# MAC-VO/MAC-VO

Measured on NVIDIA H100. Metric: stereo frames/sec @640x480, higher is better.
Workload: dtype f32

## Files before the change

### include/macvo_b200.h

```cpp
#ifndef MACVO_B200_H
#define MACVO_B200_H

#include <stddef.h>
#include <stdint.h>

#ifdef __cplusplus
extern "C" {
#endif

#define MACVO_OK 0
#define MACVO_E_ARG (-1)
#define MACVO_E_WORKSPACE (-2)
#define MACVO_E_UNSUPPORTED (-3)
#define MACVO_E_DRIVER (-4)

const char* macvo_b200_version(void);

#define MACVO_CORR_SIMT 0
#define MACVO_CORR_TC_3XF16 1
#define MACVO_CORR_TC_1XF16 2
#define MACVO_CORR_TC_TF32 3
#define MACVO_CORR_KMAJOR_INPUT 16
size_t macvo_corr_workspace_bytes(int batch, int dim, int n, int mode);
int macvo_corr_build(const float* fmap1, const float* fmap2, float* corr, int batch, int dim, int n, int mode,
// ... 87 lines not shown
int macvo_p2p_alloc(size_t bytes, void** dev_ptr, unsigned char* ipc_handle64);
int macvo_p2p_open(const unsigned char* ipc_handle64, void** peer_ptr);
int macvo_p2p_close(void* peer_ptr);
int macvo_p2p_free(void* dev_ptr);
int macvo_pgo_solve_sharded(const double* pos_Tw, const double* kp2_uv, const double* kp2_disp, const double* uv_cov,
                            const double* disp_cov, int k_shard, const int* k_total_dev, int k_offset, int min_k,
                            const double* intr, double* pose_io, const macvo_pgo_params_t* params, double* stats,
                            void* const* exchange_bufs, int world, int rank, void* stream);

#define MACVO_PGO_ACC 55
#define MACVO_PGO_MAX_RANKS 8
int macvo_pgo_accumulate(const double* pos_Tw, const double* kp2_uv, const double* kp2_disp, const double* uv_cov,
                         const double* disp_cov, int k, const double* intr, const double* pose, double huber_delta,
                         double* acc, void* stream);

int macvo_layer_norm(const float* x, const float* weight, const float* bias, float* y, long long rows,
                     int channels, float eps, void* stream);
int macvo_add_layer_norm(const float* x, const float* resid, const float* weight, const float* bias, float* sum_out,
                         float* y, long long rows, int channels, float eps, void* stream);
int macvo_mlp_tc(const float* xn, const float* resid, const float* w1, const float* b1, const float* w2, const float* b2,
                 float* out, int rows, int channels, int hidden, void* stream);
int macvo_patch_tokens_tc(const float* x, const float* w0, const float* term, const float* w2, const float* b2,
                          const float* ln_w, const float* ln_b, float* out, long long rows, int in_channels, int channels,
                          int period, float eps, void* stream);
int macvo_patch_embed_conv1(const float* maps, const float* weight, const float* bias, float* out,
                            long long n_maps, int h, int w, int allow_tf32, void* stream);
int macvo_add_rows_relu(float* x, const float* term, long long rows, int period, int channels, void* stream);
int macvo_small_attention(const float* q, const float* k, const float* v, float* out, int batch, int nq, int nk,
                          int heads, int head_dim, int q_broadcast, int allow_tf32, void* stream);

int macvo_small_attention_ex(const float* q, const float* k, const float* v, float* out, int batch, int nq, int nk,
                             int heads, int head_dim, int q_broadcast, int allow_tf32, int ldq, int ldk, int ldv,
                             const float* q_add, const float* k_add, int add_period, void* stream);

int macvo_latent_pool(const float* tokens, const float* ut, const float* wv, const float* bv, float* out,
                      long long n_maps, int nk, void* stream);

int macvo_gru_input(const float* mf, const float* agg, const float* gamma, float* buf0, float* buf1, float* buf2,
                    float* buf3, long long pixels, void* stream);
int macvo_gru_gates(const float* zr, const float* bias, const float* hx, float* z_out, float* rhx, long long pixels,
                    void* stream);
int macvo_gru_blend(const float* q, const float* bias, const float* z, float* hx, float* h_dense, long long pixels,
                    void* stream);
size_t macvo_rows_count(int batch, int height, int width, int vertical);
int macvo_conv_tc(const void* in_rows, int in_channels, int in_dense, const void* weights, const float* bias, int n_pad,
                  int n_valid, int ksize, int relu, int batch, int height, int width, void* out16, int out16_pitch,
                  int out16_offset, int out16_dense, float* out32, int out32_pitch, int out32_offset, int out32_planes,
                  void* stream);
int macvo_flow_im2col(const float* coords1, const float* coords0, void* rows, float* mf32, void* mf16_rows, int batch,
                      int height, int width, void* stream);

size_t macvo_gru_tc_operand_rows(int batch, int height, int width, int vertical);
int macvo_gru_tc_stage(int stage, int vertical, int batch, int height, int width, const void* h_rows, const void* x_rows,
                       const void* weights, const float* bias, float* h_master, float* z, void* out_rows, void* stream);
int macvo_gru_tc_pack(const float* src, int src_pitch, int channels, void* dst, int dst_channels, int dst_offset, int batch,
                      int height, int width, int vertical, void* stream);
int macvo_gru_tc_pack_motion(const float* mf, const float* agg, const float* gamma, void* x_rows_h, void* x_rows_v, int batch,
                             int height, int width, void* stream);
int macvo_softmax_rows_f16(const float* scores, void* out, long long rows, int cols, void* stream);
int macvo_convex_upsample(const float* flow, const float* mask_nhwc, float* out, float scale, int batch, int height, int width,
                          void* stream);

int macvo_cov_sanity_filter(const double* obs1_cov, const double* obs2_cov, int k, uint8_t* good, void* stream);
#define MACVO_COV_MATCH 0
#define MACVO_COV_IDENTITY 1
#define MACVO_COV_GAUSSIAN_MIXTURE 2
// ... 55 lines not shown
```

### mac-vo_b200/csrc/nn_kernels.cu

```cuda
#include "common.cuh"
#include "layer_norm_row.cuh"
#include <math_constants.h>

namespace {

__device__ __forceinline__ float2 ffma2_rn(float2 a, float2 b, float2 c) { return make_float2(fmaf(a.x, b.x, c.x), fmaf(a.y, b.y, c.y)); }
__device__ __forceinline__ float2 fmul2_rn(float2 a, float2 b) { return make_float2(__fmul_rn(a.x, b.x), __fmul_rn(a.y, b.y)); }

template <int VPL>
__global__ void __launch_bounds__(256)
layer_norm_kernel(const float* __restrict__ x, const float* __restrict__ w, const float* __restrict__ b,
                  float* __restrict__ y, long long rows, float eps, const float* __restrict__ resid = nullptr,
                  float* __restrict__ sum_out = nullptr) {
    constexpr int C = 32 * VPL;
    const long long row = (long long)blockIdx.x * 8 + (threadIdx.x >> 5);
    const int lane = threadIdx.x & 31;
    if (row >= rows) return;
    const float* xr = x + row * C;
    float v[VPL];
#pragma unroll
    for (int i = 0; i < VPL / 4; ++i) {
        float4 t = *reinterpret_cast<const float4*>(xr + (lane + 32 * i) * 4);
        if (resid) {
            const float4 r = *reinterpret_cast<const float4*>(resid + row * C + (lane + 32 * i) * 4);
// ... 472 lines not shown
        }
    }
    l0 += __shfl_xor_sync(0xffffffffu, l0, 1); l0 += __shfl_xor_sync(0xffffffffu, l0, 2);
    l1 += __shfl_xor_sync(0xffffffffu, l1, 1); l1 += __shfl_xor_sync(0xffffffffu, l1, 2);
    const float i0 = 1.f / l0, i1 = 1.f / l1;
    const int h0 = 2 * warp, h1 = h0 + 1;
    float o0[2][4], o1[2][4];
#pragma unroll
    for (int nt = 0; nt < 2; ++nt) { o0[nt][0] = o0[nt][1] = o0[nt][2] = o0[nt][3] = 0.f; o1[nt][0] = o1[nt][1] = o1[nt][2] = o1[nt][3] = 0.f; }
#pragma unroll
    for (int nd = 0; nd < KS; ++nd) {
        const uint32_t za[4] = {to_tf32(acc[nd][0] * i0), to_tf32(acc[nd][2] * i1), to_tf32(acc[nd][1] * i0), to_tf32(acc[nd][3] * i1)};
#pragma unroll
        for (int nt = 0; nt < 2; ++nt) {
            const float* w0 = wv + (long long)(h0 * LP_HD + nt * 8 + g) * LP_D + nd * 8 + 2 * t;
            const float* w1 = wv + (long long)(h1 * LP_HD + nt * 8 + g) * LP_D + nd * 8 + 2 * t;
            mma_tf32(o0[nt], za, to_tf32(__ldg(w0)), to_tf32(__ldg(w0 + 1)));
            mma_tf32(o1[nt], za, to_tf32(__ldg(w1)), to_tf32(__ldg(w1 + 1)));
        }
    }
    float* ob = out + (b * 8 + g) * (LP_HEADS * LP_HD);
#pragma unroll
    for (int nt = 0; nt < 2; ++nt) {
        const int d = nt * 8 + 2 * t;
        *reinterpret_cast<float2*>(ob + h0 * LP_HD + d) = make_float2(o0[nt][0] + __ldg(bv + h0 * LP_HD + d), o0[nt][1] + __ldg(bv + h0 * LP_HD + d + 1));
        *reinterpret_cast<float2*>(ob + h1 * LP_HD + d) = make_float2(o1[nt][2] + __ldg(bv + h1 * LP_HD + d), o1[nt][3] + __ldg(bv + h1 * LP_HD + d + 1));
    }
}

constexpr int FQ_HEADS = 8, FQ_SLOTS = 4, FQ_QPT = 2;
template <int FQ_D>
__global__ void __launch_bounds__(128)
attn_few_queries_kernel(const float* __restrict__ q, const float* __restrict__ k, const float* __restrict__ v,
                        float* __restrict__ out, long long batch, int nq, int nk, long long q_bstride, float scale) {
    const long long b = (long long)blockIdx.x * 4 + (threadIdx.x >> 5);
    if (b >= batch) return;
    const int lane = threadIdx.x & 31, hd = lane & 7, slot = lane >> 3;
    constexpr int C = FQ_HEADS * FQ_D;
    float2 qr[FQ_QPT][FQ_D / 2], acc[FQ_QPT][FQ_D / 2];
    float m[FQ_QPT], l[FQ_QPT];
#pragma unroll
    for (int t = 0; t < FQ_QPT; ++t) {
        const int i = min(slot + FQ_SLOTS * t, nq - 1);
        const float* qp = q + b * q_bstride + ((long long)i * FQ_HEADS + hd) * FQ_D;
#pragma unroll
        for (int c = 0; c < FQ_D / 4; ++c) {
            const float4 x = *reinterpret_cast<const float4*>(qp + 4 * c);
            qr[t][2 * c] = make_float2(x.x * scale, x.y * scale);
            qr[t][2 * c + 1] = make_float2(x.z * scale, x.w * scale);
        }
#pragma unroll
        for (int c = 0; c < FQ_D / 2; ++c) acc[t][c] = make_float2(0.f, 0.f);
        m[t] = -CUDART_INF_F; l[t] = 0.f;
    }
    const float4* kp = reinterpret_cast<const float4*>(k + b * nk * C + hd * FQ_D);
    const float4* vp = reinterpret_cast<const float4*>(v + b * nk * C + hd * FQ_D);
#pragma unroll 2
    for (int j = 0; j < nk; ++j) {
        float4 kk[FQ_D / 4], vv[FQ_D / 4];
#pragma unroll
        for (int c = 0; c < FQ_D / 4; ++c) { kk[c] = __ldg(kp + j * (C / 4) + c); vv[c] = __ldg(vp + j * (C / 4) + c); }
#pragma unroll
        for (int t = 0; t < FQ_QPT; ++t) {
            float2 sx = make_float2(0.f, 0.f);
#pragma unroll
            for (int c = 0; c < FQ_D / 4; ++c) {
                sx = ffma2_rn(qr[t][2 * c], make_float2(kk[c].x, kk[c].y), sx);
                sx = ffma2_rn(qr[t][2 * c + 1], make_float2(kk[c].z, kk[c].w), sx);
            }
            const float s = sx.x + sx.y;
            const float mn = fmaxf(m[t], s);
            const float corr = __expf(m[t] - mn), p = __expf(s - mn);
            m[t] = mn;
            l[t] = l[t] * corr + p;
            const float2 c2 = make_float2(corr, corr), p2 = make_float2(p, p);
#pragma unroll
            for (int c = 0; c < FQ_D / 4; ++c) {
                acc[t][2 * c] = ffma2_rn(p2, make_float2(vv[c].x, vv[c].y), fmul2_rn(acc[t][2 * c], c2));
                acc[t][2 * c + 1] = ffma2_rn(p2, make_float2(vv[c].z, vv[c].w), fmul2_rn(acc[t][2 * c + 1], c2));
            }
        }
    }
#pragma unroll
    for (int t = 0; t < FQ_QPT; ++t) {
        const int i = slot + FQ_SLOTS * t;
        if (i >= nq) continue;
        const float inv = 1.f / l[t];
        float* op = out + ((b * nq + i) * FQ_HEADS + hd) * FQ_D;
#pragma unroll
        for (int c = 0; c < FQ_D / 4; ++c)
            *reinterpret_cast<float4*>(op + 4 * c) = make_float4(acc[t][2 * c].x * inv, acc[t][2 * c].y * inv,
                                                                 acc[t][2 * c + 1].x * inv, acc[t][2 * c + 1].y * inv);
    }
}

template <int D>
__global__ void __launch_bounds__(256)
attn_single_query_kernel(const float* __restrict__ q, const float* __restrict__ k, const float* __restrict__ v,
                         float* __restrict__ out, long long batch, int nk, int heads, float scale) {
    const long long e = (long long)blockIdx.x * blockDim.x + threadIdx.x;
    if (e >= batch * heads) return;
    const long long b = e / heads;
    const int hd = (int)(e % heads), C = heads * D;
    float qr[D], acc[D];
#pragma unroll
    for (int c = 0; c < D; c += 4) {
        const float4 t = *reinterpret_cast<const float4*>(q + b * C + hd * D + c);
        qr[c] = t.x * scale; qr[c + 1] = t.y * scale; qr[c + 2] = t.z * scale; qr[c + 3] = t.w * scale;
        acc[c] = acc[c + 1] = acc[c + 2] = acc[c + 3] = 0.f;
    }
    float m = -CUDART_INF_F, l = 0.f;
    const float* kp = k + b * nk * C + hd * D;
    const float* vp = v + b * nk * C + hd * D;
#pragma unroll 4
    for (int j = 0; j < nk; ++j) {
        float kk[D], vv[D];
#pragma unroll
        for (int c = 0; c < D; c += 4) {
            const float4 t = __ldg(reinterpret_cast<const float4*>(kp + (long long)j * C + c));
            const float4 u = __ldg(reinterpret_cast<const float4*>(vp + (long long)j * C + c));
            kk[c] = t.x; kk[c + 1] = t.y; kk[c + 2] = t.z; kk[c + 3] = t.w;
// ... 67 lines not shown
        return MACVO_OK;
    }
    float* packed = nullptr;
    MACVO_CUDA_TRY(cudaGetSymbolAddress(reinterpret_cast<void**>(&packed), g_pe_pack));
    pe_pack_weights_kernel<<<3, 256, 0, st>>>(weight, bias, packed);
    MACVO_LAUNCH_CHECK();
    MACVO_CUDA_TRY(cudaMemcpyToSymbolAsync(c_pe_w, packed, sizeof(float) * (PE_K * PE_K * PE_C + PE_C), 0,
                                           cudaMemcpyDeviceToDevice, st));
    MACVO_CUDA_TRY(cudaFuncSetAttribute(patch_conv1_kernel, cudaFuncAttributeMaxDynamicSharedMemorySize, (int)smem));
    const int items = ho * (wo / 2);
    patch_conv1_kernel<<<(unsigned)n_maps, items % 320 == 0 ? 320 : 256, smem, st>>>(maps, out, h, w, ho, wo);
    MACVO_LAUNCH_CHECK();
    return MACVO_OK;
}

extern "C" int macvo_small_attention_ex(const float* q, const float* k, const float* v, float* out, int batch, int nq,
                                        int nk, int heads, int head_dim, int q_broadcast, int allow_tf32, int ldq, int ldk,
                                        int ldv, const float* q_add, const float* k_add, int add_period, void* stream) {
    if (!q || !k || !v || !out || batch <= 0 || nq <= 0 || nk <= 0 || heads <= 0) return MACVO_E_ARG;
    if (head_dim != 8 && head_dim != 16 && head_dim != 32) return MACVO_E_UNSUPPORTED;
    const int c = heads * head_dim;
    AttnExtra ex{ldq > 0 ? ldq : c, ldk > 0 ? ldk : c, ldv > 0 ? ldv : c, add_period > 0 ? add_period : 1, q_add, k_add};
    const bool plain = ex.ldq == c && ex.ldk == c && ex.ldv == c && !q_add && !k_add;
    if ((ex.ldq | ex.ldk | ex.ldv) & 3) return MACVO_E_ARG;
    cudaStream_t st = as_stream(stream);
    const float scale = 1.f / sqrtf((float)head_dim);
    const long long qbs = q_broadcast ? 0 : (long long)nq * ex.ldq;
    if (plain && nq == 1 && !q_broadcast && head_dim <= 16) {
        const unsigned grid = (unsigned)(((long long)batch * heads + 255) / 256);
        if (head_dim == 16) attn_single_query_kernel<16><<<grid, 256, 0, st>>>(q, k, v, out, batch, nk, heads, scale);
        else attn_single_query_kernel<8><<<grid, 256, 0, st>>>(q, k, v, out, batch, nk, heads, scale);
    } else if (plain && nq <= FQ_SLOTS * FQ_QPT && heads == FQ_HEADS && head_dim <= 16) {
        const unsigned grid = (unsigned)((batch + 3) / 4);
        if (head_dim == 16) attn_few_queries_kernel<16><<<grid, 128, 0, st>>>(q, k, v, out, batch, nq, nk, qbs, scale);
        else attn_few_queries_kernel<8><<<grid, 128, 0, st>>>(q, k, v, out, batch, nq, nk, qbs, scale);
    } else if (head_dim == 8) {
        return MACVO_E_UNSUPPORTED;
    } else if (allow_tf32 && nq >= 16) {
        const size_t smem = (size_t)((nk + 31) / 32 * 32) * ((head_dim / 32) * 32 + 16 + head_dim) * sizeof(float);
        if (smem > 200 * 1024) return MACVO_E_UNSUPPORTED;
        const int warps = nq > 64 ? 8 : 4;
        dim3 grid(ceil_div(nq, 16 * warps), heads, batch);
        if (head_dim == 16) {
            MACVO_CUDA_TRY(cudaFuncSetAttribute(attn_tc_kernel<16>, cudaFuncAttributeMaxDynamicSharedMemorySize, (int)smem));
            attn_tc_kernel<16><<<grid, 32 * warps, smem, st>>>(q, k, v, out, nq, nk, heads, qbs, scale, ex);
        } else {
            MACVO_CUDA_TRY(cudaFuncSetAttribute(attn_tc_kernel<32>, cudaFuncAttributeMaxDynamicSharedMemorySize, (int)smem));
            attn_tc_kernel<32><<<grid, 32 * warps, smem, st>>>(q, k, v, out, nq, nk, heads, qbs, scale, ex);
        }
    } else {
        const size_t smem = (size_t)2 * ((nk + ATT_CHUNK - 1) / ATT_CHUNK * ATT_CHUNK) * head_dim * sizeof(float);
        if (smem > 200 * 1024) return MACVO_E_UNSUPPORTED;
        dim3 grid(ceil_div(nq, 128), heads, batch);
        if (head_dim == 16) {
            MACVO_CUDA_TRY(cudaFuncSetAttribute(attn_shared_kv_kernel<16>, cudaFuncAttributeMaxDynamicSharedMemorySize, (int)smem));
            attn_shared_kv_kernel<16><<<grid, 128, smem, st>>>(q, k, v, out, nq, nk, heads, qbs, scale, ex);
        } else {
            MACVO_CUDA_TRY(cudaFuncSetAttribute(attn_shared_kv_kernel<32>, cudaFuncAttributeMaxDynamicSharedMemorySize, (int)smem));
            attn_shared_kv_kernel<32><<<grid, 128, smem, st>>>(q, k, v, out, nq, nk, heads, qbs, scale, ex);
        }
    }
    MACVO_LAUNCH_CHECK();
    return MACVO_OK;
}

extern "C" int macvo_small_attention(const float* q, const float* k, const float* v, float* out, int batch, int nq,
                                     int nk, int heads, int head_dim, int q_broadcast, int allow_tf32, void* stream) {
    return macvo_small_attention_ex(q, k, v, out, batch, nq, nk, heads, head_dim, q_broadcast, allow_tf32, 0, 0, 0, nullptr,
                                    nullptr, 0, stream);
}

extern "C" int macvo_add_rows_relu(float* x, const float* term, long long rows, int period, int channels, void* stream) {
    if (!x || !term || rows < 0 || period <= 0 || channels <= 0 || (channels & 3)) return MACVO_E_ARG;
    if (rows == 0) return MACVO_OK;
    const long long n = rows * (channels / 4);
    add_rows_relu_kernel<<<(unsigned)((n + 255) / 256), 256, 0, as_stream(stream)>>>(x, term, rows, period, channels / 4);
    MACVO_LAUNCH_CHECK();
    return MACVO_OK;
}

extern "C" int macvo_latent_pool(const float* tokens, const float* ut, const float* wv, const float* bv, float* out,
                                 long long n_maps, int nk, void* stream) {
    if (!tokens || !ut || !wv || !bv || !out || n_maps < 0 || nk <= 0) return MACVO_E_ARG;
    if (n_maps == 0) return MACVO_OK;
    const size_t smem = (size_t)((nk + 31) / 32 * 32) * (LP_D + 4) * sizeof(float);
    if (smem > 200 * 1024) return MACVO_E_UNSUPPORTED;
    MACVO_CUDA_TRY(cudaFuncSetAttribute(latent_pool_kernel, cudaFuncAttributeMaxDynamicSharedMemorySize, (int)smem));
    latent_pool_kernel<<<(unsigned)n_maps, 128, smem, as_stream(stream)>>>(tokens, ut, wv, bv, out, nk);
    MACVO_LAUNCH_CHECK();
    return MACVO_OK;
}
```

### mac-vo_b200/flowformer_cov.py

```python
from __future__ import annotations

import math
import os
import zlib
from typing import Callable

import torch
import torch.nn.functional as F

Tensor = torch.Tensor

LATENT_TOKENS = 8
LATENT_DIM = 128
QUERY_DIM = 64
COST_INPUT_DIM = 64
VERT_C_DIM = 64
ENCODER_DEPTH = 3


def _svt_spec(prefix: str) -> list[tuple[str, tuple[int, ...], str]]:
    out: list[tuple[str, tuple[int, ...], str]] = []
    dims, heads, srs, patch, cin = (128, 256), (4, 8), (8, 4), (4, 2), (3, 128)
    for s, (C, sr, ps, ci) in enumerate(zip(dims, srs, patch, cin)):
        p = f"{prefix}.svt."
# ... 348 lines not shown
                x = self._ops.patch_embed_conv1(cost_maps, self.W[p + "proj.0.weight"], self.W[p + "proj.0.bias"])
                x = self._conv_relu(x, p + "proj.2", stride=2, padding=2)
        else:
            x = F.pad(cost_maps, (0, (8 - W2 % 8) % 8, 0, (8 - H2 % 8) % 8))
            x = self._conv_relu(x, p + "proj.0", stride=2, padding=2)
            x = self._conv_relu(x, p + "proj.2", stride=2, padding=2)
        native = self._native(x)
        x = F.conv2d(x if x.is_contiguous(memory_format=torch.channels_last) else x.contiguous(memory_format=torch.channels_last),
                     self.W[p + "proj.4.weight"], None if native else self.W[p + "proj.4.bias"], stride=2, padding=2)
        h, w = x.shape[2:]

        w0, b0 = self.W[p + "ffn_with_coord.0.weight"], self.W[p + "ffn_with_coord.0.bias"]

        def coord_term():
            xy = coords_grid(1, h, w, x.device, x.dtype) * 8 + 4
            enc = sine_embed(xy.view(1, 2, -1).permute(0, 2, 1), COST_INPUT_DIM)
            term = F.linear(enc, w0[:, COST_INPUT_DIM:, 0, 0], b0)
            if native:
                term = term + F.linear(self.W[p + "proj.4.bias"], w0[:, :COST_INPUT_DIM, 0, 0])
            return term.contiguous()
        term = self._memo(("pe", h, w, x.dtype, x.device, native), coord_term)
        t = x.permute(0, 2, 3, 1).reshape(M, h * w, COST_INPUT_DIM)
        w2 = self.W[p + "ffn_with_coord.2.weight"][:, :, 0, 0]
        if native and torch.backends.cuda.matmul.allow_tf32:
            w0t, w2t = self._memo(("pe_tc", x.device), lambda: (self._ops.round_tf32(w0[:, :COST_INPUT_DIM, 0, 0]),
                                                                self._ops.round_tf32(w2)))
            return self._ops.patch_tokens_tc(t, w0t, term[0], w2t, self.W[p + "ffn_with_coord.2.bias"],
                                             self.W[p + "norm.weight"], self.W[p + "norm.bias"])
        t = F.linear(t, w0[:, :COST_INPUT_DIM, 0, 0])
        t = self._ops.add_rows_relu_(t, term[0]) if native else F.relu(t + term)
        t = F.linear(t, w2, self.W[p + "ffn_with_coord.2.bias"])
        return self._ln(t, p + "norm")

    def _latent_layer(self, x: Tensor, p: str) -> Tensor:
        y = self._ln(x, p + "norm1")
        a = self._attn(self._lin(y, p + "q"), self._lin(y, p + "k"), self._lin(y, p + "v"), 8)
        x, xn = self._add_ln(x, self._lin(a, p + "proj"), p + "norm2")
        return self._mlp_residual(x, xn, p, "ffn.0", "ffn.3")

    def _context_tokens(self, context: Tensor, p: str, reps: int) -> Tensor:
        b, _, H, W = context.shape
        c = self._lin(context.flatten(2).permute(0, 2, 1), p + "context_proj").view(b, H, W, -1)
        return c.repeat(reps, 1, 1, 1)

    def _vert_local_attn_native(self, x: Tensor, size, context: Tensor, p: str, ws: int, heads: int) -> Tensor:
        Bt, N, C = x.shape
        H, W = size
        b = context.shape[0]
        wq, wk = self.W[p + "q.weight"], self.W[p + "k.weight"]
        enc = self._memo(("win", ws, C + VERT_C_DIM, x.dtype, x.device), lambda: sine_embed(
            coords_grid(1, ws, ws, x.device, x.dtype).view(1, 2, -1).permute(0, 2, 1), C + VERT_C_DIM))
        cproj = self._lin(context.flatten(2).permute(0, 2, 1), p + "context_proj").view(b, H, W, -1)
        cw, meta = self._to_windows(cproj, ws)
        w_qk_c = torch.cat([wq[:, C:], wk[:, C:]], 0)
        w_qk = torch.cat([wq, wk], 0)
        b_qk = torch.cat([self.W[p + "q.bias"], self.W[p + "k.bias"]], 0)
        terms = F.linear(cw, w_qk_c) + F.linear(enc, w_qk, b_qk)
        q_add, k_add = terms[..., :C].contiguous(), terms[..., C:].contiguous()
        w_x = self._memo(("vloc_w", p), lambda: torch.cat([wq[:, :C], wk[:, :C], self.W[p + "v.weight"]], 0).contiguous())
        b_x = self._memo(("vloc_b", p), lambda: torch.cat([torch.zeros(2 * C, device=x.device, dtype=x.dtype), self.W[p + "v.bias"]], 0))
        xw, meta = self._to_windows(x.view(Bt, H, W, C), ws)
        qkv = F.linear(xw, w_x, b_x)
        o = self._ops.fused_qkv_attention(qkv, heads, q_add, k_add)
        return self._lin(self._from_windows(o, meta, ws, H, W), p + "proj")

    def _vert_local_attn(self, x: Tensor, size, context: Tensor, p: str, ws: int = 7, heads: int = 8) -> Tensor:
        if self._native(x) and (x.shape[-1] // heads) in (16, 32):
            return self._vert_local_attn_native(x, size, context, p, ws, heads)
        Bt, N, C = x.shape
        H, W = size
        ctx = self._context_tokens(context, p, Bt // context.shape[0])
# ... 51 lines not shown
        k_in = self._conv(qk.permute(0, 3, 1, 2), p + "sr_key", stride=sr).reshape(Bt, C, -1).permute(0, 2, 1)
        v_in, k_in = self._ln(v_in, p + "norm"), self._ln(k_in, p + "norm")
        enc_sub = self._memo(("sub", Hp // sr, Wp // sr, sr, C, x.dtype, x.device), lambda: sine_embed(
            coords_grid(1, Hp // sr, Wp // sr, x.device, x.dtype).view(1, 2, -1).permute(0, 2, 1) * sr, C))
        o = self._attn(q, self._lin(k_in + enc_sub, p + "k"), self._lin(v_in, p + "v"), heads)
        o = o.view(Bt, Hp, Wp, C)[:, :H, :W, :].reshape(Bt, N, C)
        return self._lin(o, p + "proj")

    def _vert_block(self, x: Tensor, size, context: Tensor, p: str, local: bool) -> Tensor:
        attn = self._vert_local_attn if local else self._vert_global_attn
        x, xn = self._add_ln(x, attn(self._ln(x, p + "norm1"), size, context, p + "attn."), p + "norm2")
        return self._mlp_residual(x, xn, p + "mlp.", "fc1", "fc2")

    def cost_perceiver(self, cost_volume: Tensor, context: Tensor) -> tuple[Tensor, Tensor]:
        c = "memory_encoder.cost_perceiver_encoder."
        B, heads, H1, W1, H2, W2 = cost_volume.shape
        assert heads == 1
        cost_maps = cost_volume.view(B * H1 * W1, 1, H2, W2)
        tokens = self.patch_embed(cost_maps)
        p = c + "input_layer."
        lat = self.W[c + "latent_tokens"]
        M = tokens.shape[0]
        q = self._lin(self._ln(lat, p + "norm1"), p + "q")
        if self._native(tokens) and torch.backends.cuda.matmul.allow_tf32 and LATENT_DIM == 128 and LATENT_TOKENS == 8:
            a = self._ops.latent_pool(tokens, q[0], self.W[p + "k.weight"], self.W[p + "v.weight"], self.W[p + "v.bias"])
        else:
            a = self._attn(q, self._lin(tokens, p + "k"), self._lin(tokens, p + "v"), 8)
        x = lat + self._lin(a, p + "proj")
        x = self._mlp_residual(x, self._ln(x, p + "norm2"), p, "ffn.0", "ffn.3")
        short_cut = x
        N = H1 * W1
        self._join_context()
        for i in range(ENCODER_DEPTH):
            x = self._latent_layer(x, c + f"encoder_layers.{i}.")
            x = x.view(B, N, LATENT_TOKENS, -1).permute(0, 2, 1, 3).reshape(B * LATENT_TOKENS, N, -1)
            v_ = c + f"vertical_encoder_layers.{i}."
            x = self._vert_block(x, (H1, W1), context, v_ + "local_block.", True)
            x = self._vert_block(x, (H1, W1), context, v_ + "global_block.", False)
            x = x.view(B, LATENT_TOKENS, N, -1).permute(0, 2, 1, 3).reshape(B * N, LATENT_TOKENS, -1)
        return x + short_cut, cost_maps

    def memory_encoder(self, img1: Tensor, img2: Tensor, context: Tensor, shared: tuple[int, int] | None = None) -> tuple[Tensor, Tensor]:
        B = img1.shape[0]
        if shared is None:
            feats = self.svt(torch.cat([img1, img2], dim=0), "memory_encoder.feat_encoder")
            feats = self._conv(feats, "memory_encoder.channel_convertor")
            f1, f2 = feats[:B], feats[B:]
        else:
            i, j = shared
            if not (0 <= i < B and 0 <= j < B):
                raise ValueError(f"shared={shared}: image indices must lie in [0, {B})")
            keep = [k for k in range(B) if k != j]
            feats = self.svt(torch.cat([img1] + [img2[k:k + 1] for k in keep], dim=0), "memory_encoder.feat_encoder")
            feats = self._conv(feats, "memory_encoder.channel_convertor")
            f1 = feats[:B]
            f2 = torch.empty_like(f1)
            for pos, k in enumerate(keep):
                f2[k:k + 1].copy_(feats[B + pos:B + pos + 1])
            f2[j:j + 1].copy_(feats[i:i + 1])
            if self.taps is not None:
                feats = torch.cat([f1, f2], dim=0)
        self._tap("feats", feats)
        cost_volume = self.corr_fn(f1, f2).to(feats.dtype)
        self._tap("corr_rows", cost_volume.reshape(B, -1, cost_volume.shape[-2] * cost_volume.shape[-1])[:, ::97])
        out = self.cost_perceiver(cost_volume, context)
        self._tap("cost_memory", out[0])
        return out

    def _gru(self, h: Tensor, x: Tensor, p: str) -> Tensor:
        for o, pad in (("1", (0, 2)), ("2", (2, 0))):
            hx = torch.cat([h, x], dim=1)
            zr = torch.sigmoid(self._conv(hx, p + f"convzr{o}", padding=pad))
# ... 316 lines not shown
```

### mac-vo_b200/ops.py

```python
from __future__ import annotations

import ctypes as C
import os
import threading

import torch

from .build import LIB_PATH

Tensor = torch.Tensor
F32, F64 = torch.float32, torch.float64

CORR_SIMT, CORR_TC_3XF16, CORR_TC_1XF16, CORR_TC_TF32 = 0, 1, 2, 3
CORR_MODE_NAMES = {0: "simt", 1: "tc3", 2: "tc1", 3: "tf32"}
CORR_KMAJOR_INPUT = 16
PGO_ACC = 55

_lib = None
_lock = threading.Lock()
LAUNCHES = [0]


class MacvoB200Error(RuntimeError):
    pass
# ... 43 lines not shown
                                          + [C.c_float] * 4 + [C.c_int] + [C.c_float] * 2 + [C.c_void_p] * 4),
    "macvo_pgo_solve": (C.c_int, [C.c_void_p] * 5 + [C.c_int] + [C.c_void_p] * 2 + [C.POINTER(_PgoParams)]
                        + [C.c_void_p] * 2),
    "macvo_pgo_solve_graph": (C.c_int, [C.c_int] + [C.c_void_p] * 8 + [C.c_int] + [C.c_void_p] * 2 + [C.POINTER(_PgoParams)]
                              + [C.c_void_p] * 2),
    "macvo_pgo_solve_counted": (C.c_int, [C.c_void_p] * 5 + [C.c_int, C.c_void_p, C.c_int] + [C.c_void_p] * 2
                                + [C.POINTER(_PgoParams)] + [C.c_void_p] * 2 + [C.c_int] + [C.c_void_p] * 3),
    "macvo_motion_interpolate_workspace_bytes": (C.c_size_t, [C.c_int]),
    "macvo_motion_interpolate": (C.c_int, [C.c_void_p, C.c_void_p, C.c_int, C.c_void_p, C.c_void_p, C.c_size_t, C.c_void_p]),
    "macvo_cov_sanity_filter": (C.c_int, [C.c_void_p] * 2 + [C.c_int] + [C.c_void_p] * 2),
    "macvo_cov_modify": (C.c_int, [C.c_void_p, C.c_int, C.c_void_p, C.c_int, C.c_void_p]),
    "macvo_observe_workspace_bytes": (C.c_size_t, [C.c_int]),
    "macvo_observe_packed_doubles": (C.c_size_t, [C.c_int, C.c_int]),
    "macvo_observe_pack": (C.c_int, [C.c_void_p, C.c_int, C.c_int] + [C.c_void_p] * 6 + [C.c_int] * 3 + [C.c_void_p] * 2
                           + [C.c_int] + [C.c_float] * 3 + [C.c_void_p] * 6 + [C.c_size_t, C.c_void_p]
                           + [C.POINTER(_ObserveExt)]),
    "macvo_pgo_exchange_bytes": (C.c_size_t, [C.c_int]),
    "macvo_p2p_alloc": (C.c_int, [C.c_size_t, C.POINTER(C.c_void_p), C.c_char_p]),
    "macvo_p2p_open": (C.c_int, [C.c_char_p, C.POINTER(C.c_void_p)]),
    "macvo_p2p_close": (C.c_int, [C.c_void_p]),
    "macvo_p2p_free": (C.c_int, [C.c_void_p]),
    "macvo_pgo_solve_sharded": (C.c_int, [C.c_void_p] * 5 + [C.c_int, C.c_void_p, C.c_int, C.c_int] + [C.c_void_p] * 2
                                + [C.POINTER(_PgoParams)] + [C.c_void_p] * 2 + [C.c_int, C.c_int, C.c_void_p]),
    "macvo_pgo_accumulate": (C.c_int, [C.c_void_p] * 5 + [C.c_int] + [C.c_void_p] * 2 + [C.c_double]
                             + [C.c_void_p] * 2),
    "macvo_layer_norm": (C.c_int, [C.c_void_p] * 4 + [C.c_longlong, C.c_int, C.c_float, C.c_void_p]),
    "macvo_add_layer_norm": (C.c_int, [C.c_void_p] * 6 + [C.c_longlong, C.c_int, C.c_float, C.c_void_p]),
    "macvo_mlp_tc": (C.c_int, [C.c_void_p] * 7 + [C.c_int] * 3 + [C.c_void_p]),
    "macvo_patch_tokens_tc": (C.c_int, [C.c_void_p] * 8 + [C.c_longlong, C.c_int, C.c_int, C.c_int, C.c_float, C.c_void_p]),
    "macvo_patch_embed_conv1": (C.c_int, [C.c_void_p] * 4 + [C.c_longlong, C.c_int, C.c_int, C.c_int, C.c_void_p]),
    "macvo_add_rows_relu": (C.c_int, [C.c_void_p] * 2 + [C.c_longlong, C.c_int, C.c_int, C.c_void_p]),
    "macvo_small_attention": (C.c_int, [C.c_void_p] * 4 + [C.c_int] * 7 + [C.c_void_p]),
    "macvo_small_attention_ex": (C.c_int, [C.c_void_p] * 4 + [C.c_int] * 10 + [C.c_void_p] * 2 + [C.c_int, C.c_void_p]),
    "macvo_latent_pool": (C.c_int, [C.c_void_p] * 5 + [C.c_longlong, C.c_int, C.c_void_p]),
    "macvo_decoder_token_blob_floats": (C.c_size_t, []),
    "macvo_decoder_token": (C.c_int, [C.c_void_p] * 6 + [C.c_int, C.c_int, C.c_float, C.c_void_p]),
    "macvo_decoder_token_rows": (C.c_int, [C.c_void_p] * 6 + [C.c_int] * 3 + [C.c_float, C.c_void_p]),
    "macvo_gru_input": (C.c_int, [C.c_void_p] * 7 + [C.c_longlong, C.c_void_p]),
    "macvo_gru_gates": (C.c_int, [C.c_void_p] * 5 + [C.c_longlong, C.c_void_p]),
    "macvo_gru_blend": (C.c_int, [C.c_void_p] * 5 + [C.c_longlong, C.c_void_p]),
    "macvo_softmax_rows_f16": (C.c_int, [C.c_void_p] * 2 + [C.c_longlong, C.c_int, C.c_void_p]),
    "macvo_convex_upsample": (C.c_int, [C.c_void_p] * 3 + [C.c_float] + [C.c_int] * 3 + [C.c_void_p]),
    "macvo_rows_count": (C.c_size_t, [C.c_int] * 4),
    "macvo_conv_tc": (C.c_int, [C.c_void_p, C.c_int, C.c_int, C.c_void_p, C.c_void_p] + [C.c_int] * 7
                      + [C.c_void_p] + [C.c_int] * 3 + [C.c_void_p] + [C.c_int] * 3 + [C.c_void_p]),
    "macvo_flow_im2col": (C.c_int, [C.c_void_p] * 5 + [C.c_int] * 3 + [C.c_void_p]),
    "macvo_gru_tc_operand_rows": (C.c_size_t, [C.c_int] * 4),
    "macvo_gru_tc_stage": (C.c_int, [C.c_int] * 5 + [C.c_void_p] * 8),
    "macvo_gru_tc_pack": (C.c_int, [C.c_void_p, C.c_int, C.c_int, C.c_void_p] + [C.c_int] * 6 + [C.c_void_p]),
    "macvo_gru_tc_pack_motion": (C.c_int, [C.c_void_p] * 5 + [C.c_int] * 3 + [C.c_void_p]),
    "macvo_posenet_input": (C.c_int, [C.c_void_p] * 2 + [C.c_int] * 2 + [C.c_double, C.c_void_p, C.c_void_p]),
    "macvo_posenet_conv": (C.c_int, [C.c_void_p, C.c_int, C.c_int, C.c_int] + [C.c_void_p] * 2 + [C.c_int] * 5
                           + [C.c_void_p, C.c_int, C.c_void_p, C.c_void_p]),
    "macvo_posenet_head_floats": (C.c_size_t, []),
    "macvo_posenet_head": (C.c_int, [C.c_void_p] * 6),
    "macvo_pwc_warp_corr": (C.c_int, [C.c_void_p] * 3 + [C.c_float] + [C.c_int] * 4 + [C.c_void_p] + [C.c_int] * 2
                            + [C.c_void_p]),
    "macvo_stereo_head": (C.c_int, [C.c_void_p] * 3 + [C.c_int] * 2 + [C.c_void_p] * 4 + [C.c_float] * 2 + [C.c_int] * 4
                          + [C.c_void_p] * 3),
}


def load_library(path: str | None = None):
    global _lib
    with _lock:
        if _lib is not None:
# ... 643 lines not shown
                                        (ln_b, "ln_b")))
    cin, c = x.shape[-1], w0.shape[0]
    if (cin != 64 or c != 128 or tuple(w0.shape) != (c, cin) or tuple(w2.shape) != (c, c) or term.dim() != 2
            or term.shape[1] != c or term.shape[0] == 0 or any(t.numel() != c for t in (b2, ln_w, ln_b))):
        raise MacvoB200Error(f"patch_tokens_tc: unsupported shapes x {tuple(x.shape)}, w0 {tuple(w0.shape)}, "
                             f"term {tuple(term.shape)}, w2 {tuple(w2.shape)}")
    out = torch.empty(*x.shape[:-1], c, dtype=torch.float32, device=x.device)
    _launch("macvo_patch_tokens_tc", x, w0, term, w2, b2, ln_w, ln_b, out, x.numel() // cin, cin, c, term.shape[0], float(eps))
    return out


def patch_embed_conv1(maps: Tensor, weight: Tensor, bias: Tensor, allow_tf32: bool | None = None, s2d: bool = False) -> Tensor:
    maps = _arg(maps, F32, "patch_embed_conv1 maps", copy=True)
    m, one, h, w = maps.shape
    if one != 1 or tuple(weight.shape) != (16, 1, 6, 6):
        raise MacvoB200Error("patch_embed_conv1: expects (M,1,H,W) maps and a (16,1,6,6) weight")
    ho, wo = (h + 7) // 8 * 4, (w + 7) // 8 * 4
    tf32 = bool(torch.backends.cudnn.allow_tf32 if allow_tf32 is None else allow_tf32)
    if s2d and not tf32:
        raise MacvoB200Error("patch_embed_conv1: the space-to-depth output exists for the TF32 tensor-core variant only")
    out = torch.empty((m, ho // 2, wo // 2, 64) if s2d else (m, ho, wo, 16), dtype=torch.float32, device=maps.device)
    _launch("macvo_patch_embed_conv1", maps, _arg(weight, F32, "patch_embed_conv1 weight", copy=True),
            _arg(bias, F32, "patch_embed_conv1 bias", copy=True), out, m, h, w, int(tf32) | (2 if s2d else 0))
    return out.permute(0, 3, 1, 2)


def space_to_depth_filter(weight: Tensor) -> Tensor:
    o, c, kh, kw = weight.shape
    if (kh, kw) != (6, 6):
        raise MacvoB200Error("space_to_depth_filter: expects a 6x6 filter")
    return weight.reshape(o, c, 3, 2, 3, 2).permute(0, 3, 5, 1, 2, 4).reshape(o, 4 * c, 3, 3)


def small_attention(q: Tensor, k: Tensor, v: Tensor, heads: int, allow_tf32: bool | None = None) -> Tensor:
    if allow_tf32 is None:
        allow_tf32 = bool(torch.backends.cuda.matmul.allow_tf32)
    q, k, v = (_arg(t, F32, f"small_attention {n}", copy=True) for t, n in ((q, "q"), (k, "k"), (v, "v")))
    b, nk, c = k.shape
    d = c // heads
    nq = q.shape[1]
    if q.shape[0] not in (1, b) or q.shape[2] != c or v.shape != k.shape or d * heads != c:
        raise MacvoB200Error(f"small_attention: bad shapes q{tuple(q.shape)} k{tuple(k.shape)} v{tuple(v.shape)}")
    out = torch.empty(b, nq, c, dtype=torch.float32, device=k.device)
    _launch("macvo_small_attention", q, k, v, out, b, nq, nk, heads, d, int(q.shape[0] == 1 and b > 1), int(allow_tf32))
    return out


GRU_HID, GRU_IN = 128, 512


def gru_input(mf: Tensor, agg: Tensor, gamma: Tensor, bufs: list[Tensor]) -> None:
    mf, agg = _arg(mf, F32, "gru_input mf", cols=GRU_HID), _arg(agg, F32, "gru_input agg", cols=GRU_HID)
    bufs = [_arg(b, F32, "gru_input buffer", shape=(None, GRU_IN)) for b in bufs] + [None] * (4 - len(bufs))
    _launch("macvo_gru_input", mf, agg, _arg(gamma, F32, "gru_input gamma", copy=True), *bufs, mf.numel() // GRU_HID)


def gru_gates(zr: Tensor, hx: Tensor, z_out: Tensor, rhx: Tensor, bias: Tensor | None = None) -> None:
    _launch("macvo_gru_gates", _arg(zr, F32, "gru_gates zr", cols=2 * GRU_HID),
            _arg(bias, F32, "gru_gates bias", numel=2 * GRU_HID, optional=True),
            _arg(hx, F32, "gru_gates hx", shape=(None, GRU_IN)), _arg(z_out, F32, "gru_gates z_out", cols=GRU_HID),
            _arg(rhx, F32, "gru_gates rhx", shape=(None, GRU_IN)), hx.shape[0])


def gru_blend(q: Tensor, z: Tensor, hx: Tensor, h_dense: Tensor | None, bias: Tensor | None = None) -> None:
    _launch("macvo_gru_blend", _arg(q, F32, "gru_blend q", cols=GRU_HID),
            _arg(bias, F32, "gru_blend bias", numel=GRU_HID, optional=True), _arg(z, F32, "gru_blend z", cols=GRU_HID),
            _arg(hx, F32, "gru_blend hx", shape=(None, GRU_IN)),
            _arg(h_dense, F32, "gru_blend h_dense", cols=GRU_HID, optional=True), hx.shape[0])


# ... 355 lines not shown
```

Measured before the change: 47.48.

## Run latent attention directly on vertical token layout to skip permute copies

Measured after the change: 47.81 (median of 6 runs). No clear change (+0.7%).

```diff
diff --git a/include/macvo_b200.h b/include/macvo_b200.h
--- a/include/macvo_b200.h
+++ b/include/macvo_b200.h
@@ -143,6 +143,9 @@
 int macvo_small_attention_ex(const float* q, const float* k, const float* v, float* out, int batch, int nq, int nk,
                              int heads, int head_dim, int q_broadcast, int allow_tf32, int ldq, int ldk, int ldv,
                              const float* q_add, const float* k_add, int add_period, void* stream);
+
+int macvo_small_attention_interleaved(const float* q, const float* k, const float* v, float* out, int images, int pixels,
+                                      int tokens, int heads, int head_dim, void* stream);
 
 int macvo_latent_pool(const float* tokens, const float* ut, const float* wv, const float* bv, float* out,
                       long long n_maps, int nk, void* stream);
diff --git a/mac-vo_b200/csrc/nn_kernels.cu b/mac-vo_b200/csrc/nn_kernels.cu
--- a/mac-vo_b200/csrc/nn_kernels.cu
+++ b/mac-vo_b200/csrc/nn_kernels.cu
@@ -528,17 +528,20 @@
 template <int FQ_D>
 __global__ void __launch_bounds__(128)
 attn_few_queries_kernel(const float* __restrict__ q, const float* __restrict__ k, const float* __restrict__ v,
-                        float* __restrict__ out, long long batch, int nq, int nk, long long q_bstride, float scale) {
+                        float* __restrict__ out, long long batch, int nq, int nk, long long q_bstride, float scale,
+                        long long g) {
     const long long b = (long long)blockIdx.x * 4 + (threadIdx.x >> 5);
     if (b >= batch) return;
     const int lane = threadIdx.x & 31, hd = lane & 7, slot = lane >> 3;
     constexpr int C = FQ_HEADS * FQ_D;
+    const long long bg = b / g, bi = b - bg * g;
     float2 qr[FQ_QPT][FQ_D / 2], acc[FQ_QPT][FQ_D / 2];
     float m[FQ_QPT], l[FQ_QPT];
 #pragma unroll
     for (int t = 0; t < FQ_QPT; ++t) {
         const int i = min(slot + FQ_SLOTS * t, nq - 1);
-        const float* qp = q + b * q_bstride + ((long long)i * FQ_HEADS + hd) * FQ_D;
+        const long long qrow = q_bstride ? bg * nq * g + bi + i * g : i;
+        const float* qp = q + qrow * C + hd * FQ_D;
 #pragma unroll
         for (int c = 0; c < FQ_D / 4; ++c) {
             const float4 x = *reinterpret_cast<const float4*>(qp + 4 * c);
@@ -549,13 +552,13 @@
         for (int c = 0; c < FQ_D / 2; ++c) acc[t][c] = make_float2(0.f, 0.f);
         m[t] = -CUDART_INF_F; l[t] = 0.f;
     }
-    const float4* kp = reinterpret_cast<const float4*>(k + b * nk * C + hd * FQ_D);
-    const float4* vp = reinterpret_cast<const float4*>(v + b * nk * C + hd * FQ_D);
+    const float4* kp = reinterpret_cast<const float4*>(k + (bg * nk * g + bi) * C + hd * FQ_D);
+    const float4* vp = reinterpret_cast<const float4*>(v + (bg * nk * g + bi) * C + hd * FQ_D);
 #pragma unroll 2
     for (int j = 0; j < nk; ++j) {
         float4 kk[FQ_D / 4], vv[FQ_D / 4];
 #pragma unroll
-        for (int c = 0; c < FQ_D / 4; ++c) { kk[c] = __ldg(kp + j * (C / 4) + c); vv[c] = __ldg(vp + j * (C / 4) + c); }
+        for (int c = 0; c < FQ_D / 4; ++c) { kk[c] = __ldg(kp + j * g * (C / 4) + c); vv[c] = __ldg(vp + j * g * (C / 4) + c); }
 #pragma unroll
         for (int t = 0; t < FQ_QPT; ++t) {
             float2 sx = make_float2(0.f, 0.f);
@@ -582,7 +585,7 @@
         const int i = slot + FQ_SLOTS * t;
         if (i >= nq) continue;
         const float inv = 1.f / l[t];
-        float* op = out + ((b * nq + i) * FQ_HEADS + hd) * FQ_D;
+        float* op = out + (bg * nq * g + bi + i * g) * C + hd * FQ_D;
 #pragma unroll
         for (int c = 0; c < FQ_D / 4; ++c)
             *reinterpret_cast<float4*>(op + 4 * c) = make_float4(acc[t][2 * c].x * inv, acc[t][2 * c].y * inv,
@@ -716,8 +719,8 @@
         else attn_single_query_kernel<8><<<grid, 256, 0, st>>>(q, k, v, out, batch, nk, heads, scale);
     } else if (plain && nq <= FQ_SLOTS * FQ_QPT && heads == FQ_HEADS && head_dim <= 16) {
         const unsigned grid = (unsigned)((batch + 3) / 4);
-        if (head_dim == 16) attn_few_queries_kernel<16><<<grid, 128, 0, st>>>(q, k, v, out, batch, nq, nk, qbs, scale);
-        else attn_few_queries_kernel<8><<<grid, 128, 0, st>>>(q, k, v, out, batch, nq, nk, qbs, scale);
+        if (head_dim == 16) attn_few_queries_kernel<16><<<grid, 128, 0, st>>>(q, k, v, out, batch, nq, nk, qbs, scale, 1);
+        else attn_few_queries_kernel<8><<<grid, 128, 0, st>>>(q, k, v, out, batch, nq, nk, qbs, scale, 1);
     } else if (head_dim == 8) {
         return MACVO_E_UNSUPPORTED;
     } else if (allow_tf32 && nq >= 16) {
@@ -754,6 +757,21 @@
                                     nullptr, 0, stream);
 }
 
+extern "C" int macvo_small_attention_interleaved(const float* q, const float* k, const float* v, float* out, int images,
+                                                 int pixels, int tokens, int heads, int head_dim, void* stream) {
+    if (!q || !k || !v || !out || images <= 0 || pixels <= 0 || tokens <= 0 || heads <= 0) return MACVO_E_ARG;
+    if (tokens > FQ_SLOTS * FQ_QPT || heads != FQ_HEADS || (head_dim != 8 && head_dim != 16)) return MACVO_E_UNSUPPORTED;
+    const long long batch = (long long)images * pixels;
+    const unsigned grid = (unsigned)((batch + 3) / 4);
+    const float scale = 1.f / sqrtf((float)head_dim);
+    const long long qbs = (long long)tokens * heads * head_dim;
+    cudaStream_t st = as_stream(stream);
+    if (head_dim == 16) attn_few_queries_kernel<16><<<grid, 128, 0, st>>>(q, k, v, out, batch, tokens, tokens, qbs, scale, pixels);
+    else attn_few_queries_kernel<8><<<grid, 128, 0, st>>>(q, k, v, out, batch, tokens, tokens, qbs, scale, pixels);
+    MACVO_LAUNCH_CHECK();
+    return MACVO_OK;
+}
+
 extern "C" int macvo_add_rows_relu(float* x, const float* term, long long rows, int period, int channels, void* stream) {
     if (!x || !term || rows < 0 || period <= 0 || channels <= 0 || (channels & 3)) return MACVO_E_ARG;
     if (rows == 0) return MACVO_OK;
diff --git a/mac-vo_b200/flowformer_cov.py b/mac-vo_b200/flowformer_cov.py
--- a/mac-vo_b200/flowformer_cov.py
+++ b/mac-vo_b200/flowformer_cov.py
@@ -404,11 +404,22 @@
         t = F.linear(t, w2, self.W[p + "ffn_with_coord.2.bias"])
         return self._ln(t, p + "norm")
 
-    def _latent_layer(self, x: Tensor, p: str) -> Tensor:
+    def _latent_layer(self, x: Tensor, p: str, B: int, N: int, in_vertical: bool) -> Tensor:
+        C = x.shape[-1]
+        to_vertical = lambda t: t.view(B, N, LATENT_TOKENS, C).permute(0, 2, 1, 3).reshape(B * LATENT_TOKENS, N, C)
+        if self._native(x) and LATENT_TOKENS == 8 and C in (64, 128):
+            if not in_vertical:
+                x = to_vertical(x)
+            y = self._ln(x, p + "norm1")
+            a = self._ops.small_attention(self._lin(y, p + "q"), self._lin(y, p + "k"), self._lin(y, p + "v"), 8, interleaved=True)
+            x, xn = self._add_ln(x, self._lin(a, p + "proj"), p + "norm2")
+            return self._mlp_residual(x, xn, p, "ffn.0", "ffn.3")
+        if in_vertical:
+            x = x.view(B, LATENT_TOKENS, N, C).permute(0, 2, 1, 3).reshape(B * N, LATENT_TOKENS, C)
         y = self._ln(x, p + "norm1")
         a = self._attn(self._lin(y, p + "q"), self._lin(y, p + "k"), self._lin(y, p + "v"), 8)
         x, xn = self._add_ln(x, self._lin(a, p + "proj"), p + "norm2")
-        return self._mlp_residual(x, xn, p, "ffn.0", "ffn.3")
+        return to_vertical(self._mlp_residual(x, xn, p, "ffn.0", "ffn.3"))
 
     def _context_tokens(self, context: Tensor, p: str, reps: int) -> Tensor:
         b, _, H, W = context.shape
@@ -526,12 +537,11 @@
         N = H1 * W1
         self._join_context()
         for i in range(ENCODER_DEPTH):
-            x = self._latent_layer(x, c + f"encoder_layers.{i}.")
-            x = x.view(B, N, LATENT_TOKENS, -1).permute(0, 2, 1, 3).reshape(B * LATENT_TOKENS, N, -1)
+            x = self._latent_layer(x, c + f"encoder_layers.{i}.", B, N, in_vertical=i > 0)
             v_ = c + f"vertical_encoder_layers.{i}."
             x = self._vert_block(x, (H1, W1), context, v_ + "local_block.", True)
             x = self._vert_block(x, (H1, W1), context, v_ + "global_block.", False)
-            x = x.view(B, LATENT_TOKENS, N, -1).permute(0, 2, 1, 3).reshape(B * N, LATENT_TOKENS, -1)
+        x = x.view(B, LATENT_TOKENS, N, -1).permute(0, 2, 1, 3).reshape(B * N, LATENT_TOKENS, -1)
         return x + short_cut, cost_maps
 
     def memory_encoder(self, img1: Tensor, img2: Tensor, context: Tensor, shared: tuple[int, int] | None = None) -> tuple[Tensor, Tensor]:
diff --git a/mac-vo_b200/ops.py b/mac-vo_b200/ops.py
--- a/mac-vo_b200/ops.py
+++ b/mac-vo_b200/ops.py
@@ -99,6 +99,7 @@
     "macvo_add_rows_relu": (C.c_int, [C.c_void_p] * 2 + [C.c_longlong, C.c_int, C.c_int, C.c_void_p]),
     "macvo_small_attention": (C.c_int, [C.c_void_p] * 4 + [C.c_int] * 7 + [C.c_void_p]),
     "macvo_small_attention_ex": (C.c_int, [C.c_void_p] * 4 + [C.c_int] * 10 + [C.c_void_p] * 2 + [C.c_int, C.c_void_p]),
+    "macvo_small_attention_interleaved": (C.c_int, [C.c_void_p] * 4 + [C.c_int] * 5 + [C.c_void_p]),
     "macvo_latent_pool": (C.c_int, [C.c_void_p] * 5 + [C.c_longlong, C.c_int, C.c_void_p]),
     "macvo_decoder_token_blob_floats": (C.c_size_t, []),
     "macvo_decoder_token": (C.c_int, [C.c_void_p] * 6 + [C.c_int, C.c_int, C.c_float, C.c_void_p]),
@@ -808,10 +809,20 @@
     return weight.reshape(o, c, 3, 2, 3, 2).permute(0, 3, 5, 1, 2, 4).reshape(o, 4 * c, 3, 3)
 
 
-def small_attention(q: Tensor, k: Tensor, v: Tensor, heads: int, allow_tf32: bool | None = None) -> Tensor:
+def small_attention(q: Tensor, k: Tensor, v: Tensor, heads: int, allow_tf32: bool | None = None,
+                    interleaved: bool = False) -> Tensor:
     if allow_tf32 is None:
         allow_tf32 = bool(torch.backends.cuda.matmul.allow_tf32)
     q, k, v = (_arg(t, F32, f"small_attention {n}", copy=True) for t, n in ((q, "q"), (k, "k"), (v, "v")))
+    if interleaved:
+        rows, p, c = k.shape
+        tokens = 8 if rows % 8 == 0 else 0
+        if q.shape != k.shape or v.shape != k.shape or heads != 8 or c not in (64, 128) or not tokens:
+            raise MacvoB200Error(f"small_attention: interleaved operands must be (images * 8, pixels, 8 heads x 8 or 16) "
+                                 f"alike, got q{tuple(q.shape)} k{tuple(k.shape)} v{tuple(v.shape)} with {heads} heads")
+        out = torch.empty_like(k)
+        _launch("macvo_small_attention_interleaved", q, k, v, out, rows // tokens, p, tokens, heads, c // heads)
+        return out
     b, nk, c = k.shape
     d = c // heads
     nq = q.shape[1]
```
